# eriq-augustine/KB2E

Hardware: AMD Instinct MI355X
Metric: training triples/sec (1/2/4/8 MI355X) + FB15k Hits@10(Filter) (higher is better)
Workload: dtype f64

## Files before the change

kb2e_amd/csrc/engine.hip:

```cpp
#include <hip/hip_runtime.h>
#include <hip/hip_ext.h>
#include <hipcub/hipcub.hpp>

#include <algorithm>
#include <cmath>
#include <cstdio>
#include <cstring>
#include <map>
#include <memory>
#include <stdexcept>
#include <string>
#include <vector>

#include "../../include/kb2e_engine.h"
#include "glibc_rand.hpp"
#include "hip_util.hpp"
#include "eval.hpp"
#include "predict.hpp"
#include "classify.hpp"
#include "host_data.hpp"
#include "kernels_common.hpp"
#include "kernels_index.hpp"
#include "kernels_transe.hpp"
#include "kernels_transe_long.hpp"
// ... 1606 lines not shown
            for (int g = 0; g < 2; ++g) {
                fprintf(stderr, "fold_prof %d", g);
                for (int k = 0; k < 16; ++k) fprintf(stderr, " %llu", fp[g][k]);
                fprintf(stderr, "\n");
            }
            std::memset(fp, 0, sizeof(fp));
            HIPCHK(hipMemcpyToSymbol(HIP_SYMBOL(g_fold_prof), fp, sizeof(fp)));
            HIPCHK(hipMemcpyFromSymbol(fp[0], HIP_SYMBOL(g_long_prof), sizeof(fp[0])));
            fprintf(stderr, "long_prof");
            for (int k = 0; k < 16; ++k) fprintf(stderr, " %llu", fp[0][k]);
            fprintf(stderr, "\n");
            HIPCHK(hipMemcpyToSymbol(HIP_SYMBOL(g_long_prof), fp[1], sizeof(fp[1])));
        }
#endif
        if (getenv("KB2E_RPAR_STATS")) {
            unsigned long long st[16];
            HIPCHK(hipMemcpyFromSymbol(st, HIP_SYMBOL(g_rpar_rounds), sizeof(st)));
            cons_wave_take_stats(st);
            fprintf(stderr, "rpar_rounds rounds of row blocks %llu, tiles with violators %llu, most rounds of a block %llu\n",
                    st[0], st[1], st[2]);
            fprintf(stderr, "rpar_cons cycles: setup %llu, P0+rounds %llu, records %llu, longest block %llu, blocks %llu\n",
                    st[3], st[4], st[5], st[6], st[7]);
            if (c->rpar_cons_seq || c->rpar_cons_wide) {
                unsigned long long q[64];
                cons_seq_take_stats(q);
                fprintf(stderr, "rpar_cons chunk kernel: relations %llu, chunks %llu (most in a relation %llu), "
                        "violators %llu, rounds %llu (most %llu), cycles mean %.0f max %llu\n", q[0], q[1], q[6], q[2],
                        q[3], q[7], q[0] ? (double)q[4] / (double)q[0] : 0.0, q[5]);
                if (c->rpar_cons_wide && cons_chainw_pipelined(c->n))
                    fprintf(stderr, "rpar_cons pipelined wide chain phases (walker: prologue+K0, window list, walk, "
                            "B1 wait, row stores+fold, B2 wait, drain, window flags, tail, write-back+records, -; helper: "
                            "debt+fold+B2, X tile, B1 wait; walker: row+V, sums+rounds+g, later rows):");
                else if (c->rpar_cons_wide)
                    fprintf(stderr, "rpar_cons wide chain phases (prologue, window list, rows+barrier, P+Gram+B1, "
                            "K0, V+sums, B(1), rounds+g, B(2), later pairs, B(3), records+W update, chunk barrier, "
                            "window flags, tail, write-back):");
                else
                    fprintf(stderr, "rpar_cons chunk phases (prologue, chunk start, walk end + publish, B1 wait, "
                            "pick + row to LDS, helper B1 wait, after B1, V, sums, rounds + g, g store, later rows; helper wave 1: debt, tiles, "
                            "helper_sync wait, rows + corrections):");
                for (int k = 8; k < 24; ++k) fprintf(stderr, " %llu", q[k]);
                fprintf(stderr, "; hot relations (%llu, %llu chunks, %llu violators):", q[41], q[40], q[42]);
                for (int k = 24; k < 40; ++k) fprintf(stderr, " %llu", q[k]);
                if (c->rpar_cons_seq) {
                    fprintf(stderr, "; tail (last debt + barrier, slices to LDS + barrier, records, W write-back):");
                    for (int k = 44; k < 48; ++k) fprintf(stderr, " %llu", q[k]);
                    fprintf(stderr, "; hot tail:");
                    for (int k = 48; k < 52; ++k) fprintf(stderr, " %llu", q[k]);
                    fprintf(stderr, "; hot cycles %llu", q[43]);
                }
                fprintf(stderr, "\n");
            }
            if (c->rpar_cons_wave)
                fprintf(stderr, "rpar_cons wave kernel: longest setup %llu, P0+rounds %llu, records %llu, a wave's "
                        "rounds %llu; MFMA rounds before the VALU tail %llu, blocks entering it %llu\n",
                        st[8], st[9], st[10], st[11], st[12], st[13]);
            else
                fprintf(stderr, "rpar_rounds wave 0: loads+mfma issue %llu, barriers %llu, update part %llu, lockstep "
                        "rounds %llu, tail %llu, G+ballot %llu\n", st[8], st[9], st[10], st[11], st[12], st[13]);
            std::memset(st, 0, sizeof(st));
            HIPCHK(hipMemcpyToSymbol(HIP_SYMBOL(g_rpar_rounds), st, sizeof(st)));
        }
        if (loss) *loss = c->acc_loss;
        if (active) *active = c->acc_active;
        c->acc_loss = 0;
        c->acc_active = 0;
        return KB2E_OK;
    });
}

kb2e_status kb2e_train_epoch(kb2e_ctx* c, double* loss, int64_t* active) {
    return guarded(c, [&] {
// ... 288 lines not shown
```

kb2e_amd/csrc/engine_transr_parallel.inc:

```
namespace {

constexpr int32_t kRParLongMin = 128;

template <typename T, bool P, bool G>
const void* tile_fn(int nb) {
    switch (nb) {
        case 1: return (const void*)transr_tile_mfma_kernel<T, P, G, 1>;
        case 2: return (const void*)transr_tile_mfma_kernel<T, P, G, 2>;
        case 3: return (const void*)transr_tile_mfma_kernel<T, P, G, 3>;
        case 4: return (const void*)transr_tile_mfma_kernel<T, P, G, 4>;
        case 5: return (const void*)transr_tile_mfma_kernel<T, P, G, 5>;
        case 6: return (const void*)transr_tile_mfma_kernel<T, P, G, 6>;
        case 7: return (const void*)transr_tile_mfma_kernel<T, P, G, 7>;
        case 8: return (const void*)transr_tile_mfma_kernel<T, P, G, 8>;
    }
    throw std::runtime_error("TransR tile kernel: n > 128");
}

template <typename T>
const void* cons_tile_fn(int nb) {
    switch (nb) {
        case 1: return (const void*)transr_cons_tile_kernel<T, 1>;
        case 2: return (const void*)transr_cons_tile_kernel<T, 2>;
        case 3: return (const void*)transr_cons_tile_kernel<T, 3>;
// ... 269 lines not shown
        d.ne = c->cfg.num_entities;
        d.B = (int32_t)c->B;
        d.kl = c->kl;
        d.si = c->si_[set].as<int32_t>();
        d.sj = c->sj_[set].as<int32_t>();
        d.side = c->side_[set].as<uint8_t>();
        d.heads = c->heads.as<int32_t>();
        d.tails = c->tails.as<int32_t>();
        d.batch_t0 = c->rpar_batch_t0.as<int32_t>();
        d.td_r = c->rpar_td_r.as<int32_t>();
        d.td_cnt = c->rpar_td_cnt.as<int32_t>();
        d.td_kk = c->rpar_td_kk.as<int32_t>();
        d.td_ent = c->rpar_td_ent.as<int32_t>();
        rtile_desc_kernel<<<2048, 256, 0, st>>>(d);
        HIPCHK(hipGetLastError());
    }
}

DevBuf& buf_set(int set, DevBuf& s0, DevBuf& s1) { return set ? s1 : s0; }

bool sub_overlap_on() {
    const char* e = getenv("KB2E_SUB_OVERLAP");
    return !(e && e[0] == '0');
}

template <typename T>
void fill_rpar(kb2e_ctx* c, int64_t b, int j, int set, RParArgs& a, RParBufs<T>& bf) {
    const int64_t ib = b * c->sub + j;
    const int64_t first = b * c->B + (int64_t)j * c->Bs;
    const int64_t cnt = std::min<int64_t>(c->Bs, c->B - (int64_t)j * c->Bs);
    a = RParArgs{};
    a.heads = c->heads.as<int32_t>();
    a.tails = c->tails.as<int32_t>();
    a.rels = c->rels.as<int32_t>();
    a.si = c->si() + first;
    a.sj = c->sj() + first;
    a.side = c->side() + first;
    a.B = (int32_t)cnt;
    a.n = c->n;
    a.ld = c->ld;
    a.ne = c->cfg.num_entities;
    a.nr = c->cfg.num_relations;
    a.St = c->rpar_St;
    a.tgroup = c->rpar_tgroup;
    a.batch = (int32_t)ib;
    a.lr = c->cfg.learning_rate;
// ... 26 lines not shown
    bf.W = c->w.as<T>();
    bf.x = buf_set(set, c->xreal, c->sb_x).as<T>();
    bf.d = buf_set(set, c->aux, c->sb_d).as<T>();
    bf.y = buf_set(set, c->rpar_y, c->sb_y).as<T>();
    bf.wpart = buf_set(set, c->rpar_wpart, c->sb_wpart).as<T>();
    bf.rpart = buf_set(set, c->rpar_rpart, c->sb_rpart).as<T>();
    bf.pair = c->rpar_pair.as<T>();
    bf.relpair = c->rpar_relpair.as<T>();
    bf.relpair_stamp = c->rpar_relpair_stamp.as<uint32_t>();
    bf.err = c->dataflow_err.as<uint32_t>() + 1;
    if (c->rpar_mfma) {
        bf.pflag = buf_set(set, c->rpar_pflag, c->sb_pflag).as<uint8_t>();
        bf.cons_tile = buf_set(set, c->rpar_cons_tile, c->sb_cons_tile).as<int32_t>();
        bf.cons_ppt = c->rpar_cons_wave ? kConsPpt : 1;
        bf.cpairs = buf_set(set, c->rpar_cpairs, c->sb_cpairs).as<int32_t>();
        bf.vio = buf_set(set, c->rpar_vio, c->sb_vio).as<int32_t>();
        bf.cnrows = buf_set(set, c->rpar_cnrows, c->sb_cnrows).as<int32_t>();
        bf.stats = getenv("KB2E_RPAR_STATS") != nullptr;
        bf.last_renorm = c->rpar_cons_seq ? 1 : 0;
        if (const char* dbg = getenv("KB2E_CONS_DBG")) bf.dbg = atoi(dbg);
        if (const char* cl = getenv("KB2E_RPAR_CHAIN_LIST")) bf.chain_list = std::max(64, atoi(cl));
        if (const char* ct = getenv("KB2E_RPAR_CHAIN_TILES")) bf.chain_tiles = std::max(1, atoi(ct));
        if (const char* rc = getenv("KB2E_RPAR_REC_CAP")) bf.rec_cap = std::max(4, atoi(rc));
    }
    if (c->rpar_cons_wide || c->rpar_cons_gen || c->rpar_widep) {
        bf.pflag = buf_set(set, c->rpar_pflag, c->sb_pflag).as<uint8_t>();
        if (const char* dbg = getenv("KB2E_CONS_DBG")) bf.dbg = atoi(dbg);
        bf.stats = getenv("KB2E_RPAR_STATS") != nullptr;
        bf.last_renorm = 1;
    }
}

template <typename T>
void transr_phase_b(kb2e_ctx* c, RParArgs a, RParBufs<T> bf);

template <typename T>
void run_subbatch_transr_parallel(kb2e_ctx* c, int64_t b, int j) {
    const bool ov = c->sub > 1 && sub_overlap_on();
    const bool side = ov && j > 0;
    const int set = ov ? (j & 1) : 0;
    hipStream_t sa = side ? c->suba_stream : c->stream;
    RParArgs a;
    RParBufs<T> bf;
    fill_rpar<T>(c, b, j, set, a, bf);
    {
        unsigned long long* t0 = c->rpar_ptab.as<unsigned long long>();
// ... 225 lines not shown
```

kb2e_amd/csrc/kernels_transr_parallel.hpp:

```cpp
#pragma once

#include <type_traits>

#include "kernels_common.hpp"

namespace kb2e {

struct RTile {
    int32_t seg, q;
};

struct RParArgs {
    const int32_t* heads;
    const int32_t* tails;
    const int32_t* rels;
    const int32_t* si;
    const int32_t* sj;
    const uint8_t* side;
    int32_t B, n, ld, ne, nr, St;
    int32_t batch;
    int32_t tgroup;
    double lr, margin;
    int32_t compat, l1;
    const uint64_t* keys;
// ... 121 lines not shown
    T* ent;
    T* rel;
    T* W;
    T* x;
    T* d;
    T* y;
    T* wpart;
    T* rpart;
    T* pair;
    T* relpair;
    uint32_t* relpair_stamp;
    uint32_t stamp;
    uint8_t* pflag;
    int32_t* cons_tile;
    int32_t cons_ppt;
    int32_t* cpairs;
    int32_t* cnrows;
    int32_t stats;
    int32_t last_renorm;
    int32_t dbg;
    int32_t chain_list;
    int32_t chain_tiles;
    int32_t rec_cap;
    int32_t* vio;
    uint32_t* err;
};

__host__ __device__ constexpr int rm_up16_host_dev(int v) { return (v + 15) & ~15; }
constexpr int kCPairs = 64;

struct RParMerge {
    int32_t sub;
    int32_t Bs;
    int32_t Blast;
    int32_t tcap;
    int32_t nch;
    int32_t brel_cap;
};

template <typename P>
__host__ __device__ __forceinline__ void rpar_advance(P*& p, int64_t k) {
    if (p) p += k;
}

template <typename T>
__host__ __device__ __forceinline__ void rpar_sub_view(RParArgs& a, RParBufs<T>& bf, const RParMerge& m, int j) {
    const int64_t s0 = (int64_t)j * m.Bs, t0 = (int64_t)j * m.tcap;
    a.B = j == m.sub - 1 ? m.Blast : m.Bs;
    a.batch += j;
// ... 1030 lines not shown
```

kb2e_amd/csrc/kernels_transr_pipe.hpp:

```cpp
#pragma once

#include "kernels_transr_cons.hpp"
#include "kernels_transr_seq.hpp"

namespace kb2e {

constexpr int kPipeList = 1536;

template <typename T>
__host__ __device__ constexpr size_t pipe_lds(int n) {
    return sizeof(T) * ((size_t)rm_np(n) * rm_ld(n) + 5 * (size_t)kChainRows * rm_ld(n) +
                        3 * (size_t)kChainRows * (kChainRows + 1) + 4 * kChainRows + 4 * (size_t)rm_np(n)) +
           sizeof(int) * (size_t)(2 * kPipeList + kSeqMaxTiles + 1 + 8 + 2 * kChainRows);
}

constexpr int kRecGroup = 32;
constexpr int kRecReads = 8;

template <typename T, int NP, int L, int STAGE>
__device__ __forceinline__ void pipe_records(const RParArgs& a, const RParBufs<T>& bf, int r, const int32_t* vio,
                                             int nvt, const T* Wc, T* stage, int* slots, const int* slist,
                                             int nslist) {
    typedef T T2 __attribute__((ext_vector_type(2)));
    constexpr int NW = kChainThreads / kWave;
    constexpr int CAPW = STAGE / (NW * NP);
    static_assert(CAPW >= 1 && NW * CAPW <= kPipeList, "the record slots borrow a window list");
    static_assert(NP % 4 == 0 && (L * sizeof(T)) % 16 == 0 && (NP * sizeof(T)) % 16 == 0, "16-byte LDS reads");
    const int n = a.n, ld = a.ld, w = threadIdx.x >> 6, l = lane_id();
    const int nmine = nvt > w ? (nvt - w + NW - 1) / NW : 0;
    if (nmine == 0) return;
    const int capw = bf.rec_cap >= NW && bf.rec_cap < NW * CAPW ? bf.rec_cap / NW : CAPW;
    T* gs = stage + w * (CAPW * NP);
    int* sl = slots + w * CAPW;
    auto row_of = [&](int s) { return s >= 0 ? bf.pair + (int64_t)s * ld : bf.relpair + (int64_t)r * ld; };
    T wr[NP];
    {
        const T2* w2 = (const T2*)(Wc + (l < NP ? l : 0) * L);
#pragma unroll
        for (int q = 0; q < NP / 2; ++q) {
            const T2 x = w2[q];
            wr[2 * q] = x.x;
            wr[2 * q + 1] = x.y;
        }
    }
    for (int m0 = 0; m0 < nmine; m0 += capw) {
        const int cnt = nmine - m0 < capw ? nmine - m0 : capw;
        for (int i = l; i < cnt; i += kWave) {
            const int k = w + NW * (m0 + i);
            sl[i] = k < nslist ? slist[k] : vio[k];
        }
        wave_lds_sync();
        for (int i0 = 0; i0 < cnt; i0 += kRecGroup) {
            const int iu = i0 + (l & (kRecGroup - 1));
            const int sv = sl[iu < cnt ? iu : cnt - 1];
            T g[kRecGroup];
#pragma unroll
            for (int u = 0; u < kRecGroup; ++u) g[u] = row_of(__builtin_amdgcn_readlane(sv, u))[l < n ? l : 0];
            if (l < NP) {
#pragma unroll
                for (int u = 0; u < kRecGroup; ++u)
                    gs[(i0 + u < cnt ? i0 + u : cnt - 1) * NP + l] = l < n ? g[u] : T(0);
            }
        }
        wave_lds_sync();
        constexpr int NG = (NP / 2 + kRecReads - 1) / kRecReads, LA = NG >= 2 ? 2 : 1;
        T2 gr[NP / 2];
        auto g_load = [&](int i, int gq) {
            const T2* g2 = (const T2*)(gs + i * NP);
#pragma unroll
            for (int q = gq * kRecReads; q < (gq + 1) * kRecReads && q < NP / 2; ++q) gr[q] = g2[q];
        };
#pragma unroll
        for (int gq = 0; gq < LA; ++gq) g_load(0, gq);
        for (int i = 0; i < cnt; ++i) {
            T* row = row_of(sl[i]);
            const int inext = i + 1 < cnt ? i + 1 : i;
            T acc[4] = {T(0), T(0), T(0), T(0)};
            __builtin_amdgcn_sched_barrier(0);
#pragma unroll
            for (int gq = 0; gq < NG; ++gq) {
#pragma unroll
                for (int q = gq * kRecReads; q < (gq + 1) * kRecReads && q < NP / 2; ++q) {
                    acc[(2 * q) & 3] = fma(wr[2 * q], gr[q].x, acc[(2 * q) & 3]);
                    acc[(2 * q + 1) & 3] = fma(wr[2 * q + 1], gr[q].y, acc[(2 * q + 1) & 3]);
                }
                __builtin_amdgcn_sched_barrier(0);
                if (gq + LA < NG) g_load(i, gq + LA);
                else g_load(inext, gq + LA - NG);
                __builtin_amdgcn_sched_barrier(0);
            }
            T da = (acc[0] + acc[1]) + (acc[2] + acc[3]);
            asm volatile("" : "+v"(da));
            if (l < n) row[l] = -(T)a.lr * da;
        }
        wave_lds_sync();
    }
}

template <typename T, int KS, bool STATS>
__global__ __launch_bounds__(kChainThreads) void transr_cons_pipe_kernel(RParArgs a, RParBufs<T> bf) {
    using M = Mfma16<T>;
    static_assert(sizeof(T) == 8, "the D-row / k-step identity below is the FP64 fragment layout");
    constexpr int NB = (4 * KS + 15) / 16;
    constexpr int NP = 16 * NB, L = NP + 2, R = kChainRows, LG = R + 1;
    constexpr int NH = 2 * KS;
    constexpr int NSW = (NB + 2) / 3;
    static_assert(2 * R * L >= NP * L, "the K0 image borrows the two P buffers");
    static_assert(NSW * KS <= 4 * KS, "the helpers' slices share the walk's K0 registers");
    const int t0 = a.batch_t0[a.batch], t1 = a.batch_t0[a.batch + 1];
    int g0, r;
    if (!chain_first_tile(a, t0, t1, g0, r)) return;
    const int n = a.n, ld = a.ld;
    const int w = threadIdx.x >> 6, l = lane_id(), kq = l >> 4, l16 = l & 15;
    const bool mine = w < NB;
    const int col = 16 * w + l16;
    const int hw = w - 1;
    const T lr = (T)a.lr;
    extern __shared__ __attribute__((aligned(16))) char smem[];
    T* Wc = (T*)smem;
    T* Abuf = Wc + NP * L;
    T* Pbuf = Abuf + 3 * R * L;
    T* Gbuf = Pbuf + 2 * R * L;
    T* Cx = Gbuf + 2 * R * LG;
    int* slist = (int*)Cx;
    constexpr int kSlist = 2 * R * LG;
    T* qpart = Cx + R * LG;
    T* rp = qpart + 4 * R;
    int* pe = (int*)(rp + 4 * NP);
    int* ps = pe + kPipeList;
    int* pre = ps + kPipeList;
    int* misc = pre + kSeqMaxTiles + 1;
    int* vlist = misc + 8;
    const long long ck0 = STATS ? clock64() : 0;
    int n_chunks = 0;
    unsigned long long n_vio = 0, n_rounds = 0, max_m = 0;
    __shared__ unsigned long long ph[STATS ? 20 : 1];
    if (STATS && threadIdx.x < 20) ph[threadIdx.x] = 0;
    long long tq = ck0;
    auto tick = [&](int k) {
        if constexpr (STATS) {
            if (threadIdx.x == ((k >= 12 && k < 16) || k == 5 ? 64u : 0u)) {
                const long long t = clock64();
                ph[k] += (unsigned long long)(t - tq);
                tq = t;
            }
        }
    };

    for (int idx = threadIdx.x; idx < NP * NP; idx += kChainThreads) {
        const int j = idx / NP, i = idx % NP;
        Wc[j * L + i] = (j < n && i < n) ? bf.W[((int64_t)r * n + j) * ld + i] : T(0);
    }
    if (w == 0) {
        int run = 0;
        for (int m0 = 0;; m0 += kWave) {
            const int g = g0 + m0 + l;
            const uint64_t b = __ballot(t0 + g < t1 && a.td_r[t0 + g] == r);
            const int k = b == ~0ull ? kWave : __builtin_ctzll(~b);
            run += k;
            if (k < kWave) break;
        }
        const int c0 = bf.cnrows[g0] & 127;
        const int rel = c0 > 0 && bf.cpairs[(int64_t)g0 * 2 * kCPairs + kCPairs + c0 - 1] == -2;
        int kl = -1, gt = -1;
        for (int g = g0 + run - 1; g >= g0 && kl < 0; --g) {
            const int cs = a.td_cnt[t0 + g] & 255;
            const int kk = l < cs ? a.td_kk[(t0 + g) * 8 + l] : -1;
            const uint64_t b = __ballot(kk >= 0 && a.act[kk]);
            if (b) {
                kl = __shfl(kk, 63 - __builtin_clzll(b));
// ... 44 lines not shown
            for (int i = 0; i < 4 * KS; ++i) reg[i] = T(0);
#pragma unroll
            for (int si = 0; si < NSW; ++si) {
                const int cb = hw + 3 * si;
                if (cb < NB) {
#pragma unroll
                    for (int s = 0; s < KS; ++s) reg[si * KS + s] = Wc[(4 * s + kq) * L + cb * 16 + l16];
                }
            }
        }
        if (threadIdx.x == 0) {
            misc[5] = 0;
            misc[6] = -1;
            misc[7] = -1;
        }
        __syncthreads();
    }
    bool changed = false;
    int32_t* const vio = bf.vio + (int64_t)g0 * kCPairs;
    int nvt = 0;
    int pend_nv = 0, pend_par = 0, pend_pc = 0, pend_ka = 0;
    tick(0);

    auto gram_tile = [&](const T* Ar, const T* Bm, int rt, int cb, T* out, int ldo) {
        typename M::acc_t acc = {T(0), T(0), T(0), T(0)};
        T av[KS], bv[KS];
#pragma unroll
        for (int s = 0; s < KS; ++s) {
            av[s] = Ar[(rt * 16 + l16) * L + 4 * s + kq];
            bv[s] = Bm[(cb * 16 + l16) * L + 4 * s + kq];
        }
#pragma unroll
        for (int s = 0; s < KS; ++s) acc = M::mma(av[s], bv[s], acc);
#pragma unroll
        for (int q = 0; q < 4; ++q) out[(rt * 16 + kq + 4 * q) * ldo + cb * 16 + l16] = acc[q];
    };
    auto proj_tile = [&](const T* Ar, int rt, int si, T* out) {
        const int cb = hw + 3 * si;
        typename M::acc_t acc = {T(0), T(0), T(0), T(0)};
        T av[KS];
#pragma unroll
        for (int s = 0; s < KS; ++s) av[s] = Ar[(rt * 16 + l16) * L + 4 * s + kq];
#pragma unroll
        for (int s = 0; s < KS; ++s) acc = M::mma(av[s], reg[si * KS + s], acc);
#pragma unroll
        for (int q = 0; q < 4; ++q) out[(rt * 16 + kq + 4 * q) * L + cb * 16 + l16] = acc[q];
    };
    constexpr int kHT = kChainThreads - kWave;
    constexpr int kRowsPer = (R * NP + kHT - 1) / kHT;
    static_assert(kRowsPer <= 32, "rows_ok bits");
    const int ht = (int)threadIdx.x - kWave;
    T rows[kRowsPer];
    uint32_t rows_ok = 0;
    auto load_rows = [&](int b, int e) {
        if (w == 0) return;
        int ent[kRowsPer];
#pragma unroll
        for (int q = 0; q < kRowsPer; ++q) {
            const int f = b + (ht + q * kHT) / NP;
            ent[q] = pe[f < kPipeList ? f : kPipeList - 1];
        }
        rows_ok = 0;
#pragma unroll
        for (int q = 0; q < kRowsPer; ++q) {
            const int idx = ht + q * kHT;
// ... 6 lines not shown
    auto store_rows = [&](int slot) {
        if (w == 0) return;
#pragma unroll
        for (int q = 0; q < kRowsPer; ++q) {
            const int idx = ht + q * kHT;
            if (idx < R * NP) Abuf[slot * R * L + (idx / NP) * L + idx % NP] = ((rows_ok >> q) & 1) ? rows[q] : T(0);
        }
    };
    int hsync_target = 0;
    auto helper_sync = [&]() {
        hsync_target += kChainThreads / kWave - 1;
        if (l == 0 && !((bf.dbg & 32) && hw == 0))
            __hip_atomic_fetch_add(&misc[5], 1, __ATOMIC_RELEASE, __HIP_MEMORY_SCOPE_WORKGROUP);
        for (uint32_t sp = 0;
             __hip_atomic_load(&misc[5], __ATOMIC_ACQUIRE, __HIP_MEMORY_SCOPE_WORKGROUP) < hsync_target; ++sp) {
            if (sp > (1u << 22)) {
                if (l == 0) __hip_atomic_store(bf.err, 1u, __ATOMIC_RELAXED, __HIP_MEMORY_SCOPE_AGENT);
                break;
            }
            __builtin_amdgcn_s_sleep(1);
        }
    };
    auto chunk_outputs = [&](T* Pn, int cn, const T* Pc, const T* An, const T* Ac, const int* vl, int ck, int base,
                             int cc, int vpar) {
        constexpr int NE = NP / 16, NPS = (R + 11) / 12;
        const int rs = ht >> 4, cb = (ht & 15) * NE;
        T x[NPS][NE];
#pragma unroll
        for (int p = 0; p < NPS; ++p) {
            const int j = rs + 12 * p;
#pragma unroll
            for (int u = 0; u < NE; ++u) x[p][u] = j < cn ? Pn[j * L + cb + u] : T(0);
        }
        int used = 0;
        for (uint32_t sp = 0;; ++sp) {
            const bool done = __hip_atomic_load(&misc[6], __ATOMIC_ACQUIRE, __HIP_MEMORY_SCOPE_WORKGROUP) == ck;
            const int pw = __hip_atomic_load(&misc[7], __ATOMIC_ACQUIRE, __HIP_MEMORY_SCOPE_WORKGROUP);
            const int avail = (pw >> 6) == ck ? (pw & 63) : 0;
            for (; used < avail; ++used) {
                const int v = vl[used];
                const int slv = ps[base + v];
                T gv[NE], av[NE], d[NPS];
#pragma unroll
                for (int u = 0; u < NE; ++u) {
                    gv[u] = Pc[v * L + cb + u];
                    av[u] = Ac[v * L + cb + u];
                }
                if (cn > 0) {
#pragma unroll
                    for (int p = 0; p < NPS; ++p) {
                        const int j = rs + 12 * p;
                        d[p] = T(0);
#pragma unroll
                        for (int u = 0; u < NE; ++u) d[p] = fma(j < R ? An[j * L + cb + u] : T(0), av[u], d[p]);
                    }
                    row16_sums<T, NPS>(d);
#pragma unroll
                    for (int p = 0; p < NPS; ++p) {
                        const int j = rs + 12 * p;
                        if (j < cn) {
                            const T gl = -lr * d[p];
#pragma unroll
                            for (int u = 0; u < NE; ++u) x[p][u] = fma(gl, gv[u], x[p][u]);
                        }
                    }
                }
                if (rs == 0) {
                    T* dst = slv >= 0 ? bf.pair + (int64_t)slv * ld : bf.relpair + (int64_t)r * ld;
#pragma unroll
                    for (int u = 0; u < NE; ++u)
                        if (cb + u < n) dst[cb + u] = gv[u];
                    if (ht == 0) {
                        vio[nvt + used] = slv;
                        if (nvt + used < kSlist) slist[nvt + used] = slv;
                    }
                }
            }
            if (done) {
                if (ht < cc) {
                    const int sl = ps[base + ht];
                    const bool vio_l = ((uint32_t)misc[1 + 2 * vpar] >> ht) & 1;
                    if (sl >= 0) bf.pflag[sl] = vio_l ? 1 : 0;
                    else if (vio_l) bf.relpair_stamp[r] = bf.stamp;
                }
                break;
            }
            if (sp > (1u << 22)) {
                if (l == 0) __hip_atomic_store(bf.err, 1u, __ATOMIC_RELAXED, __HIP_MEMORY_SCOPE_AGENT);
                break;
            }
            __builtin_amdgcn_s_sleep(1);
        }
        if (cn == 0) return;
        T sq[NPS];
#pragma unroll
        for (int p = 0; p < NPS; ++p) {
            const int j = rs + 12 * p;
            sq[p] = T(0);
            if (j < cn) {
#pragma unroll
                for (int u = 0; u < NE; ++u) {
                    if (used) Pn[j * L + cb + u] = x[p][u];
                    sq[p] = fma(x[p][u], x[p][u], sq[p]);
                }
            }
        }
        row16_sums<T, NPS>(sq);
        if ((ht & 15) == 0) {
#pragma unroll
            for (int p = 0; p < NPS; ++p) {
                const int j = rs + 12 * p;
                if (j < R) {
                    qpart[j] = j < cn ? sq[p] : T(0);
                    for (int v = 1; v < NB; ++v) qpart[v * R + j] = T(0);
                }
            }
        }
    };
    auto correct_q = [&](T* Pn, int cn, int nv, const T* Pc, const int* vl) {
        constexpr int NE = NP / 8;
        const int j = threadIdx.x >> 3, cb = (threadIdx.x & 7) * NE;
        T sq = T(0);
        if (j < cn) {
            T x[NE];
#pragma unroll
            for (int u = 0; u < NE; ++u) x[u] = Pn[j * L + cb + u];
            for (int k = 0; k < nv; ++k) {
                const int v = vl[k];
                const T gl = -lr * Cx[j * LG + v];
#pragma unroll
                for (int u = 0; u < NE; ++u) x[u] = fma(gl, Pc[v * L + cb + u], x[u]);
            }
#pragma unroll
            for (int u = 0; u < NE; ++u) {
                if (nv) Pn[j * L + cb + u] = x[u];
                sq = fma(x[u], x[u], sq);
            }
        }
        sq += dpp_mov<0xB1>(sq);
        sq += dpp_mov<0x4E>(sq);
// ... 1 lines not shown
        if ((threadIdx.x & 7) == 0) {
            qpart[j] = j < cn ? sq : T(0);
            for (int v = 1; v < NB; ++v) qpart[v * R + j] = T(0);
        }
    };
    auto apply_pending = [&]() {
        if (w == 0 || pend_nv == 0) return;
        const T* Pp = Pbuf + pend_pc * R * L;
        const T* Ap = Abuf + pend_ka * R * L;
        const int* vl = vlist + pend_par * R;
        const int vmine = l < pend_nv ? vl[l] : 0;
        T an[KS], gn[NSW];
        auto ldv = [&](int k) {
            const int v = __builtin_amdgcn_readlane(vmine, k);
#pragma unroll
            for (int s = 0; s < KS; ++s) an[s] = Ap[v * L + 4 * s + kq];
#pragma unroll
            for (int si = 0; si < NSW; ++si) {
                const int cb = hw + 3 * si;
                gn[si] = cb < NB ? -lr * Pp[v * L + cb * 16 + l16] : T(0);
            }
        };
        const int nvu = (bf.dbg & 16) ? 0 : pend_nv;
        if (nvu > 0) ldv(0);
        for (int k = 0; k < nvu; ++k) {
            T ac[KS], gc[NSW];
#pragma unroll
            for (int s = 0; s < KS; ++s) ac[s] = an[s];
#pragma unroll
            for (int si = 0; si < NSW; ++si) gc[si] = gn[si];
            if (k + 1 < nvu) ldv(k + 1);
#pragma unroll
            for (int si = 0; si < NSW; ++si)
                if (hw + 3 * si < NB) {
#pragma unroll
                    for (int s = 0; s < KS; ++s) reg[si * KS + s] = fma(ac[s], gc[si], reg[si * KS + s]);
                }
        }
    };
    auto renorm = [&] {
        if (w > 0) {
#pragma unroll
            for (int si = 0; si < NSW; ++si) {
                const int cb = hw + 3 * si;
#pragma unroll
                for (int s = 0; s < KS; ++s) {
// ... 5 lines not shown
        }
        __syncthreads();
        if (w > 0) {
#pragma unroll
            for (int si = 0; si < NSW; ++si) {
                if (hw + 3 * si >= NB) continue;
#pragma unroll
                for (int s = 0; s < KS; ++s) {
                    const int jr = 4 * s + kq;
                    T ss = rp[jr];
                    for (int v = 1; v < NB; ++v) ss += rp[v * NP + jr];
                    if (jr < n) reg[si * KS + s] = reg[si * KS + s] / sqrt(ss);
                }
            }
        }
        __syncthreads();
    };
    auto fresh = [&](const T* A, int cc, T* P, T* G) {
        const int nrt = cc > 16 ? 2 : 1;
        if (w > 0) {
#pragma unroll
            for (int si = 0; si < NSW; ++si)
                if (hw + 3 * si < NB)
                    for (int rt = 0; rt < nrt; ++rt) proj_tile(A, rt, si, P);
        } else {
            for (int gi = 0; gi < (nrt == 2 ? 3 : 1); ++gi) gram_tile(A, A, gi == 0 ? 0 : 1, gi == 2 ? 1 : 0, G, LG);
        }
        __syncthreads();
        correct_q(P, cc, 0, nullptr, vlist);
        __syncthreads();
    };

    const int tile_cap = bf.chain_tiles >= 1 && bf.chain_tiles < kSeqMaxTiles ? bf.chain_tiles : kSeqMaxTiles;
    const int list_cap = bf.chain_list >= 64 && bf.chain_list < kPipeList ? bf.chain_list : kPipeList;
    int pc = 0;
    int par = 0;
    for (int gw = g0; gw < g0 + run || gw == g0;) {
        if (w == 0) {
            const int nt = g0 + run - gw < tile_cap ? g0 + run - gw : tile_cap;
            int carry = 0, fit = 0;
            for (int m0 = 0; m0 < nt; m0 += kWave) {
                const int g = m0 + l;
                int c = g < nt ? (bf.cnrows[gw + g] & 127) : 0;
                if (gw + g == g0 && has_rel) c -= 1;
                int x = c;
#pragma unroll
                for (int s = 1; s < kWave; s <<= 1) {
                    const int y = __shfl_up(x, s);
                    if (l >= s) x += y;
// ... 26 lines not shown
                e = cp[f - pre[lo]];
                sl = cp[kCPairs + f - pre[lo]];
            }
            pe[f] = e;
            ps[f] = sl;
        }
        auto chunk_end = [&](int b) {
            return b < tail_start ? (b + R < tail_start ? b + R : tail_start) : npairs;
        };
        __syncthreads();
        if (npairs > 0) {
            const int e0 = chunk_end(0);
            const int e1 = e0 < npairs ? chunk_end(e0) : e0;
            load_rows(0, e0);
            store_rows(0);
            load_rows(e0, e1);
            store_rows(1);
            load_rows(e1, e1 < npairs ? chunk_end(e1) : e1);
            if (tail_start == 0 && changed) renorm();
            __syncthreads();
            pc = 0;
            fresh(Abuf, e0, Pbuf, Gbuf);
        }
        int ka = 0;
        for (int base = 0; base < npairs;) {
            const int nbase = chunk_end(base);
            const int cc = nbase - base;
            const int nb2 = nbase < npairs ? chunk_end(nbase) : nbase;
            const int cn = nb2 - nbase;
            const T* A = Abuf + ka * R * L;
            const T* An = Abuf + (ka == 2 ? 0 : ka + 1) * R * L;
            T* P = Pbuf + pc * R * L;
            T* Pn = Pbuf + (pc ^ 1) * R * L;
            T* Gm = Gbuf + pc * R * LG;
            T* Gn = Gbuf + (pc ^ 1) * R * LG;
            int* vl = vlist + par * R;
            const int ck = n_chunks;
            ++n_chunks;
            tick(1);
            if (w == 0) {
                const int j = l & (R - 1);
                T q = T(0);
                if (j < cc) {
                    q = qpart[j];
                    for (int v = 1; v < NB; ++v) q += qpart[v * R + j];
                }
// ... 97 lines not shown
                                               __HIP_MEMORY_SCOPE_WORKGROUP);
                        }
                        ++npub;
                        vmask |= 1u << v;
                        cursor = v + 1;
                        if constexpr (STATS) ++n_vio;
                        tick(11);
                    }
                }
                if (l == 0) {
                    misc[1 + 2 * par] = (int)vmask;
                    misc[2 + 2 * par] = npub;
                    __hip_atomic_store(&misc[6], ck, __ATOMIC_RELEASE, __HIP_MEMORY_SCOPE_WORKGROUP);
                }
                tick(2);
            } else {
                apply_pending();
                tick(12);
                if (cn > 0) {
                    const int nrt = cn > 16 ? 2 : 1, crt = cc > 16 ? 2 : 1;
#pragma unroll
                    for (int si = 0; si < NSW; ++si)
                        if (hw + 3 * si < NB)
                            for (int rt = 0; rt < nrt; ++rt) proj_tile(An, rt, si, Pn);
                    const int ng = nrt == 2 ? 3 : 1;
                    int load[3];
#pragma unroll
                    for (int h = 0; h < 3; ++h) load[h] = nrt * ((NB - h + 2) / 3);
                    for (int tl = 0; tl < ng; ++tl) {
                        int best = 0;
#pragma unroll
                        for (int h = 1; h < 3; ++h) best = load[h] < load[best] ? h : best;
                        ++load[best];
                        if (best == hw) gram_tile(An, An, tl == 0 ? 0 : 1, tl == 2 ? 1 : 0, Gn, LG);
                    }
                    (void)crt;
                }
                tick(13);
                helper_sync();
                tick(14);
                if (nb2 < npairs || cn > 0) {
                    store_rows(ka == 0 ? 2 : ka - 1);
                    const int n3 = nb2 < npairs ? chunk_end(nb2) : nb2;
                    load_rows(n3, n3 < npairs ? chunk_end(n3) : n3);
                }
                chunk_outputs(Pn, cn, P, An, A, vl, ck, base, cc, par);
                tick(15);
            }
            __syncthreads();
            tick(w == 0 ? 3 : 5);
            const uint32_t vmask = (uint32_t)misc[1 + 2 * par];
            const int nv = misc[2 + 2 * par];
            pend_nv = nv;
            pend_par = par;
            pend_pc = pc;
            pend_ka = ka;
            nvt += nv;
            if (vmask) changed = true;
            const bool restart = nbase == tail_start && changed && cn > 0;
            tick(6);
            if (restart) {
                apply_pending();
                pend_nv = 0;
                __syncthreads();
                renorm();
                fresh(An, cn, Pn, Gn);
            }
            pc ^= 1;
            par ^= 1;
            ka = ka == 2 ? 0 : ka + 1;
            base = nbase;
        }
        apply_pending();
        pend_nv = 0;
        __syncthreads();
        tick(16);
        gw += ntile;
        if (last || gw >= g0 + run) break;
    }
    if (w > 0) {
#pragma unroll
        for (int si = 0; si < NSW; ++si) {
            const int cb = hw + 3 * si;
            if (cb < NB) {
#pragma unroll
                for (int s = 0; s < KS; ++s) Wc[(4 * s + kq) * L + cb * 16 + l16] = reg[si * KS + s];
            }
        }
    }
    __syncthreads();
    tick(17);
    pipe_records<T, NP, L, 5 * R * L>(a, bf, r, vio, nvt, Wc, Abuf, pe, slist, kSlist);
    if constexpr (STATS) {
        __syncthreads();
        tick(18);
    }
    {
        constexpr int NWB = NP * NP / kChainThreads;
        static_assert(NWB * kChainThreads == NP * NP, "whole rounds of the write-back");
        T wv[NWB];
#pragma unroll
        for (int q = 0; q < NWB; ++q) {
            const int idx = threadIdx.x + q * kChainThreads;
            wv[q] = Wc[(idx / NP) * L + idx % NP];
        }
#pragma unroll
        for (int q = 0; q < NWB; ++q) {
            const int idx = threadIdx.x + q * kChainThreads;
            const int jj = idx / NP, i = idx % NP;
            if (jj < n && i < n) bf.W[((int64_t)r * n + jj) * ld + i] = wv[q];
        }
    }
    if constexpr (STATS) {
        tick(19);
        if (threadIdx.x == 0) {
            const unsigned long long cyc = (unsigned long long)(clock64() - ck0);
            atomicAdd(&g_seq_stats[0], 1ull);
            atomicAdd(&g_seq_stats[1], (unsigned long long)n_chunks);
            atomicAdd(&g_seq_stats[2], n_vio);
            atomicAdd(&g_seq_stats[3], n_rounds);
            atomicAdd(&g_seq_stats[4], cyc);
            atomicMax(&g_seq_stats[5], cyc);
            atomicMax(&g_seq_stats[6], (unsigned long long)n_chunks);
            atomicMax(&g_seq_stats[7], max_m);
            for (int k = 0; k < 16; ++k) atomicAdd(&g_seq_stats[8 + k], ph[k]);
            for (int k = 0; k < 4; ++k) atomicAdd(&g_seq_stats[44 + k], ph[16 + k]);
            if (n_chunks >= 12) {
                for (int k = 0; k < 16; ++k) atomicAdd(&g_seq_stats[24 + k], ph[k]);
                atomicAdd(&g_seq_stats[40], (unsigned long long)n_chunks);
                atomicAdd(&g_seq_stats[41], 1ull);
                atomicAdd(&g_seq_stats[42], n_vio);
                atomicAdd(&g_seq_stats[43], cyc);
                for (int k = 0; k < 4; ++k) atomicAdd(&g_seq_stats[48 + k], ph[16 + k]);
            }
        }
    }
}

}
```

kb2e_amd/csrc/kernels_transr_seq.hpp:

```cpp
#pragma once

#include "kernels_transr_mfma.hpp"

namespace kb2e {

constexpr int kChainRows = 32;
constexpr int kChainThreads = 256;
constexpr int kSeqMaxTiles = 256;

static __device__ unsigned long long g_seq_stats[64];

template <typename T, int K>
__device__ __forceinline__ void row16_sums(T (&v)[K]) {
#pragma unroll
    for (int k = 0; k < K; ++k) v[k] += dpp_ror<8>(v[k]);
#pragma unroll
    for (int k = 0; k < K; ++k) v[k] += dpp_ror<4>(v[k]);
#pragma unroll
    for (int k = 0; k < K; ++k) v[k] += dpp_ror<2>(v[k]);
#pragma unroll
    for (int k = 0; k < K; ++k) v[k] += dpp_ror<1>(v[k]);
}

template <typename T, int K>
__device__ __forceinline__ void wave_sums(T (&v)[K]) {
    row16_sums<T, K>(v);
#pragma unroll
    for (int k = 0; k < K; ++k) v[k] += dpp_mov<kDppBcast15>(v[k]);
#pragma unroll
    for (int k = 0; k < K; ++k) v[k] += dpp_mov<kDppBcast31>(v[k]);
#pragma unroll
    for (int k = 0; k < K; ++k) v[k] = readlane_f(v[k], 63);
}
// ... 82 lines not shown
```

kb2e_amd/csrc/transr_cons.hip:

```cpp
#include "transr_cons.hpp"

#include <algorithm>
#include <cstring>
#include <stdexcept>
#include <string>
#include <utility>

#include "hip_util.hpp"
#include "kernels_transr_cons.hpp"
#include "kernels_transr_seq.hpp"
#include "kernels_transr_chainw.hpp"
#include "kernels_transr_chainwp.hpp"
#include "kernels_transr_chaing.hpp"
#include "kernels_transr_pipe.hpp"
#include "kernels_transr_wave.hpp"

namespace kb2e {

namespace {

enum Kind { kCons, kGrad, kProj, kGradMerged, kProjMerged };

int chain_grid(const RParArgs& a) { return a.nrel > 0 ? a.nrel : 1; }

// ... 178 lines not shown
    RParArgs aa = a;
    RParBufs<T> bb = bf;
    void* args[] = {&aa, &bb};
    HIPCHK(hipLaunchKernel((const void*)transr_cons_chain_gen_kernel<T>, dim3(chain_grid(a)), dim3(kGenThreads), args,
                           lds, stream));
}
template void cons_chaing_launch<double>(const RParArgs&, const RParBufs<double>&, size_t, hipStream_t);
template void cons_chaing_launch<float>(const RParArgs&, const RParBufs<float>&, size_t, hipStream_t);

template void proj_wave_launch<double>(const RParArgs&, const RParBufs<double>&, int, hipStream_t);
template void proj_wave_launch<float>(const RParArgs&, const RParBufs<float>&, int, hipStream_t);

template void grad_wave_launch<double>(const RParArgs&, const RParBufs<double>&, int, hipStream_t);
template void grad_wave_launch<float>(const RParArgs&, const RParBufs<float>&, int, hipStream_t);

template void proj_wave_merged_launch<double>(const RParArgs&, const RParBufs<double>&, const RParMerge&, hipStream_t);
template void proj_wave_merged_launch<float>(const RParArgs&, const RParBufs<float>&, const RParMerge&, hipStream_t);
template void grad_wave_merged_launch<double>(const RParArgs&, const RParBufs<double>&, const RParMerge&, hipStream_t);
template void grad_wave_merged_launch<float>(const RParArgs&, const RParBufs<float>&, const RParMerge&, hipStream_t);

template void cons_wave_launch<double>(const RParArgs&, const RParBufs<double>&, int, size_t, hipStream_t);
template void cons_wave_launch<float>(const RParArgs&, const RParBufs<float>&, int, size_t, hipStream_t);

void cons_seq_take_stats(unsigned long long (&st)[64]) {
    HIPCHK(hipMemcpyFromSymbol(st, HIP_SYMBOL(g_seq_stats), sizeof(st)));
    unsigned long long z[64] = {};
    HIPCHK(hipMemcpyToSymbol(HIP_SYMBOL(g_seq_stats), z, sizeof(z)));
}

void cons_wave_take_stats(unsigned long long (&st)[16]) {
    unsigned long long mine[16];
    HIPCHK(hipMemcpyFromSymbol(mine, HIP_SYMBOL(g_cons_stats), sizeof(mine)));
    for (int k = 0; k < 16; ++k) st[k] = (k == 2 || k == 6) ? std::max(st[k], mine[k]) : st[k] + mine[k];
    std::memset(mine, 0, sizeof(mine));
    HIPCHK(hipMemcpyToSymbol(HIP_SYMBOL(g_cons_stats), mine, sizeof(mine)));
}

}
```

kb2e_amd/csrc/transr_cons.hpp:

```cpp
#pragma once

#include <hip/hip_runtime.h>

#include "kernels_transr_parallel.hpp"

namespace kb2e {

constexpr int kWideMaxN = 112;
constexpr int kConsPpt = 1;

bool cons_wave_supported(int n);
size_t cons_wave_setup(int n, int St, int esize);
template <typename T>
void cons_wave_launch(const RParArgs& a, const RParBufs<T>& bf, int grid, size_t lds, hipStream_t stream);
template <typename T>
void proj_wave_launch(const RParArgs& a, const RParBufs<T>& bf, int grid, hipStream_t stream);
template <typename T>
void grad_wave_launch(const RParArgs& a, const RParBufs<T>& bf, int grid, hipStream_t stream);
template <typename T>
void proj_wave_merged_launch(const RParArgs& a, const RParBufs<T>& bf, const RParMerge& m, hipStream_t stream);
template <typename T>
void grad_wave_merged_launch(const RParArgs& a, const RParBufs<T>& bf, const RParMerge& m, hipStream_t stream);
size_t cons_seq_setup(int n);
void cons_seq_launch(const RParArgs& a, const RParBufs<double>& bf, size_t lds, hipStream_t stream);
bool cons_chainw_supported(int n);
size_t cons_chainw_setup(int n);
void cons_chainw_launch(const RParArgs& a, const RParBufs<double>& bf, size_t lds, hipStream_t stream);
bool cons_chaing_supported(int n);
size_t cons_chaing_setup(int n, int esize);
template <typename T>
void cons_chaing_launch(const RParArgs& a, const RParBufs<T>& bf, size_t lds, hipStream_t stream);
bool cons_chainw_pipelined(int n);
void cons_seq_take_stats(unsigned long long (&st)[64]);
void cons_wave_take_stats(unsigned long long (&st)[16]);

constexpr int kWideParMaxN = 512;
struct WideGeom {
    int St = 1;
    int chunk = 2;
    size_t tile_lds = 0, scan_lds = 0, chain_lds = 0;
};
bool wide_par_supported(int n);
WideGeom wide_setup(int n, int ld, int esize);
template <typename T>
void wide_phase_a(const RParArgs& a, const RParBufs<T>& bf, const WideGeom& g, int tgrid, double* scan,
                  double* scan_pre, const double* work_in, double* work_out, hipStream_t st);
template <typename T>
void wide_phase_b(const RParArgs& a, const RParBufs<T>& bf, const WideGeom& g, double* wsc, bool constraint,
                  int rel_segs_max, hipStream_t st);

}
```

Before: 9.449 million.

## Streamline pipelined chain handover: preload An rows, defer flags, double-buffer corrections

Adds an on-by-default pipe_opt handover mode to the pipelined TransR constraint chain kernel. The helper wave preloads its An slices into registers before polling, instead of re-reading LDS for every violator. It also stops zeroing extra qpart slots and moves the pflag/stamp writes out of the polling loop into a post-barrier step. The pending-violator correction loop is double-buffered so loads overlap FMAs, and sched barriers are placed in the MFMA tiles. Extra stats phases are added for profiling, at the cost of more register pressure and a changed write ordering for the flags.

```diff
diff --git a/kb2e_amd/csrc/engine.hip b/kb2e_amd/csrc/engine.hip
--- a/kb2e_amd/csrc/engine.hip
+++ b/kb2e_amd/csrc/engine.hip
@@ -1652,7 +1652,7 @@
             fprintf(stderr, "rpar_cons cycles: setup %llu, P0+rounds %llu, records %llu, longest block %llu, blocks %llu\n",
                     st[3], st[4], st[5], st[6], st[7]);
             if (c->rpar_cons_seq || c->rpar_cons_wide) {
-                unsigned long long q[64];
+                unsigned long long q[96];
                 cons_seq_take_stats(q);
                 fprintf(stderr, "rpar_cons chunk kernel: relations %llu, chunks %llu (most in a relation %llu), "
                         "violators %llu, rounds %llu (most %llu), cycles mean %.0f max %llu\n", q[0], q[1], q[6], q[2],
@@ -1678,6 +1678,11 @@
                     fprintf(stderr, "; hot tail:");
                     for (int k = 48; k < 52; ++k) fprintf(stderr, " %llu", q[k]);
                     fprintf(stderr, "; hot cycles %llu", q[43]);
+                    fprintf(stderr, "; hot outside the violator loop (window set-up; B1 wait at 0, 1-2, 3-5, 6+ "
+                            "violators, chunks of each; helper wave 1 after helper_sync without polling: after the walk's "
+                            "end, row staging + P_n loads, corrections + outputs; records on wave 0: W row, slot lists, "
+                            "G loads issue, arrival + staging, record loops):");
+                    for (int k = 52; k < 69; ++k) fprintf(stderr, " %llu", q[k]);
                 }
                 fprintf(stderr, "\n");
             }
diff --git a/kb2e_amd/csrc/engine_transr_parallel.inc b/kb2e_amd/csrc/engine_transr_parallel.inc
--- a/kb2e_amd/csrc/engine_transr_parallel.inc
+++ b/kb2e_amd/csrc/engine_transr_parallel.inc
@@ -315,6 +315,11 @@
 bool sub_overlap_on() {
     const char* e = getenv("KB2E_SUB_OVERLAP");
     return !(e && e[0] == '0');
+}
+
+int32_t pipe_opt_bits() {
+    const char* e = getenv("KB2E_RPAR_PIPE_OPT");
+    return e && e[0] ? (int32_t)(atoi(e) & kPipeOptAll) : kPipeOptAll;
 }
 
 template <typename T>
@@ -387,6 +392,7 @@
         if (const char* cl = getenv("KB2E_RPAR_CHAIN_LIST")) bf.chain_list = std::max(64, atoi(cl));
         if (const char* ct = getenv("KB2E_RPAR_CHAIN_TILES")) bf.chain_tiles = std::max(1, atoi(ct));
         if (const char* rc = getenv("KB2E_RPAR_REC_CAP")) bf.rec_cap = std::max(4, atoi(rc));
+        bf.pipe_opt = pipe_opt_bits();
     }
     if (c->rpar_cons_wide || c->rpar_cons_gen || c->rpar_widep) {
         bf.pflag = buf_set(set, c->rpar_pflag, c->sb_pflag).as<uint8_t>();
diff --git a/kb2e_amd/csrc/kernels_transr_parallel.hpp b/kb2e_amd/csrc/kernels_transr_parallel.hpp
--- a/kb2e_amd/csrc/kernels_transr_parallel.hpp
+++ b/kb2e_amd/csrc/kernels_transr_parallel.hpp
@@ -167,9 +167,12 @@
     int32_t chain_list;
     int32_t chain_tiles;
     int32_t rec_cap;
+    int32_t pipe_opt;
     int32_t* vio;
     uint32_t* err;
 };
+
+constexpr int32_t kPipeOptHandover = 2, kPipeOptAll = kPipeOptHandover;
 
 __host__ __device__ constexpr int rm_up16_host_dev(int v) { return (v + 15) & ~15; }
 constexpr int kCPairs = 64;
diff --git a/kb2e_amd/csrc/kernels_transr_pipe.hpp b/kb2e_amd/csrc/kernels_transr_pipe.hpp
--- a/kb2e_amd/csrc/kernels_transr_pipe.hpp
+++ b/kb2e_amd/csrc/kernels_transr_pipe.hpp
@@ -1,4 +1,6 @@
 #pragma once
+
+#include <type_traits>
 
 #include "kernels_transr_cons.hpp"
 #include "kernels_transr_seq.hpp"
@@ -17,10 +19,10 @@
 constexpr int kRecGroup = 32;
 constexpr int kRecReads = 8;
 
-template <typename T, int NP, int L, int STAGE>
+template <typename T, int NP, int L, int STAGE, bool STATS>
 __device__ __forceinline__ void pipe_records(const RParArgs& a, const RParBufs<T>& bf, int r, const int32_t* vio,
                                              int nvt, const T* Wc, T* stage, int* slots, const int* slist,
-                                             int nslist) {
+                                             int nslist, unsigned long long* ph) {
     typedef T T2 __attribute__((ext_vector_type(2)));
     constexpr int NW = kChainThreads / kWave;
     constexpr int CAPW = STAGE / (NW * NP);
@@ -29,6 +31,16 @@
     const int n = a.n, ld = a.ld, w = threadIdx.x >> 6, l = lane_id();
     const int nmine = nvt > w ? (nvt - w + NW - 1) / NW : 0;
     if (nmine == 0) return;
+    long long tq = STATS ? clock64() : 0;
+    auto tick = [&](int k) {
+        if constexpr (STATS) {
+            if (threadIdx.x == 0) {
+                const long long t = clock64();
+                ph[k] += (unsigned long long)(t - tq);
+                tq = t;
+            }
+        }
+    };
     const int capw = bf.rec_cap >= NW && bf.rec_cap < NW * CAPW ? bf.rec_cap / NW : CAPW;
     T* gs = stage + w * (CAPW * NP);
     int* sl = slots + w * CAPW;
@@ -43,6 +55,13 @@
             wr[2 * q + 1] = x.y;
         }
     }
+    if constexpr (STATS) {
+        T sink = T(0);
+#pragma unroll
+        for (int q = 0; q < NP; ++q) sink += wr[q];
+        asm volatile("" ::"v"(sink));
+    }
+    tick(0);
     for (int m0 = 0; m0 < nmine; m0 += capw) {
         const int cnt = nmine - m0 < capw ? nmine - m0 : capw;
         for (int i = l; i < cnt; i += kWave) {
@@ -50,17 +69,24 @@
             sl[i] = k < nslist ? slist[k] : vio[k];
         }
         wave_lds_sync();
+        tick(1);
         for (int i0 = 0; i0 < cnt; i0 += kRecGroup) {
             const int iu = i0 + (l & (kRecGroup - 1));
             const int sv = sl[iu < cnt ? iu : cnt - 1];
             T g[kRecGroup];
 #pragma unroll
             for (int u = 0; u < kRecGroup; ++u) g[u] = row_of(__builtin_amdgcn_readlane(sv, u))[l < n ? l : 0];
+            if constexpr (STATS) {
+                __builtin_amdgcn_sched_barrier(0);
+                tick(2);
+                __builtin_amdgcn_sched_barrier(0);
+            }
             if (l < NP) {
 #pragma unroll
                 for (int u = 0; u < kRecGroup; ++u)
                     gs[(i0 + u < cnt ? i0 + u : cnt - 1) * NP + l] = l < n ? g[u] : T(0);
             }
+            tick(3);
         }
         wave_lds_sync();
         constexpr int NG = (NP / 2 + kRecReads - 1) / kRecReads, LA = NG >= 2 ? 2 : 1;
@@ -94,6 +120,7 @@
             if (l < n) row[l] = -(T)a.lr * da;
         }
         wave_lds_sync();
+        tick(4);
     }
 }
 
@@ -134,18 +161,21 @@
     const long long ck0 = STATS ? clock64() : 0;
     int n_chunks = 0;
     unsigned long long n_vio = 0, n_rounds = 0, max_m = 0;
-    __shared__ unsigned long long ph[STATS ? 20 : 1];
-    if (STATS && threadIdx.x < 20) ph[threadIdx.x] = 0;
-    long long tq = ck0;
+    constexpr int kPh = 40;
+    __shared__ unsigned long long ph[STATS ? kPh : 1];
+    if (STATS && threadIdx.x < kPh) ph[threadIdx.x] = 0;
+    long long tq = ck0, dtq = 0;
     auto tick = [&](int k) {
         if constexpr (STATS) {
             if (threadIdx.x == ((k >= 12 && k < 16) || k == 5 ? 64u : 0u)) {
                 const long long t = clock64();
-                ph[k] += (unsigned long long)(t - tq);
+                dtq = t - tq;
+                ph[k] += (unsigned long long)dtq;
                 tq = t;
             }
         }
     };
+    const bool o_hand = (bf.pipe_opt & kPipeOptHandover) != 0;
 
     for (int idx = threadIdx.x; idx < NP * NP; idx += kChainThreads) {
         const int j = idx / NP, i = idx % NP;
@@ -236,7 +266,7 @@
     int pend_nv = 0, pend_par = 0, pend_pc = 0, pend_ka = 0;
     tick(0);
 
-    auto gram_tile = [&](const T* Ar, const T* Bm, int rt, int cb, T* out, int ldo) {
+    auto gram_tile = [&](const T* Ar, const T* Bm, int rt, int cb, T* out, int ldo, auto ahead) {
         typename M::acc_t acc = {T(0), T(0), T(0), T(0)};
         T av[KS], bv[KS];
 #pragma unroll
@@ -244,17 +274,19 @@
             av[s] = Ar[(rt * 16 + l16) * L + 4 * s + kq];
             bv[s] = Bm[(cb * 16 + l16) * L + 4 * s + kq];
         }
+        if constexpr (decltype(ahead)::value) __builtin_amdgcn_sched_barrier(0);
 #pragma unroll
         for (int s = 0; s < KS; ++s) acc = M::mma(av[s], bv[s], acc);
 #pragma unroll
         for (int q = 0; q < 4; ++q) out[(rt * 16 + kq + 4 * q) * ldo + cb * 16 + l16] = acc[q];
     };
-    auto proj_tile = [&](const T* Ar, int rt, int si, T* out) {
+    auto proj_tile = [&](const T* Ar, int rt, int si, T* out, auto ahead) {
         const int cb = hw + 3 * si;
         typename M::acc_t acc = {T(0), T(0), T(0), T(0)};
         T av[KS];
 #pragma unroll
         for (int s = 0; s < KS; ++s) av[s] = Ar[(rt * 16 + l16) * L + 4 * s + kq];
+        if constexpr (decltype(ahead)::value) __builtin_amdgcn_sched_barrier(0);
 #pragma unroll
         for (int s = 0; s < KS; ++s) acc = M::mma(av[s], reg[si * KS + s], acc);
 #pragma unroll
@@ -307,7 +339,7 @@
         }
     };
     auto chunk_outputs = [&](T* Pn, int cn, const T* Pc, const T* An, const T* Ac, const int* vl, int ck, int base,
-                             int cc, int vpar) {
+                             int cc, int vpar, long long t_sync) {
         constexpr int NE = NP / 16, NPS = (R + 11) / 12;
         const int rs = ht >> 4, cb = (ht & 15) * NE;
         T x[NPS][NE];
@@ -317,11 +349,31 @@
 #pragma unroll
             for (int u = 0; u < NE; ++u) x[p][u] = j < cn ? Pn[j * L + cb + u] : T(0);
         }
+        T anr[NPS][NE];
+#pragma unroll
+        for (int p = 0; p < NPS; ++p) {
+            const int j = rs + 12 * p;
+#pragma unroll
+            for (int u = 0; u < NE; ++u) anr[p][u] = o_hand && cn > 0 && j < R ? An[j * L + cb + u] : T(0);
+        }
         int used = 0;
+        long long tw = 0;
+        if constexpr (STATS) {
+            if (threadIdx.x == 64u) {
+                T sink = T(0);
+#pragma unroll
+                for (int p = 0; p < NPS; ++p)
+#pragma unroll
+                    for (int u = 0; u < NE; ++u) sink += x[p][u];
+                asm volatile("" ::"v"(sink));
+                ph[30] += (unsigned long long)(clock64() - t_sync);
+            }
+        }
         for (uint32_t sp = 0;; ++sp) {
             const bool done = __hip_atomic_load(&misc[6], __ATOMIC_ACQUIRE, __HIP_MEMORY_SCOPE_WORKGROUP) == ck;
             const int pw = __hip_atomic_load(&misc[7], __ATOMIC_ACQUIRE, __HIP_MEMORY_SCOPE_WORKGROUP);
             const int avail = (pw >> 6) == ck ? (pw & 63) : 0;
+            if constexpr (STATS) tw = clock64();
             for (; used < avail; ++used) {
                 const int v = vl[used];
                 const int slv = ps[base + v];
@@ -336,8 +388,13 @@
                     for (int p = 0; p < NPS; ++p) {
                         const int j = rs + 12 * p;
                         d[p] = T(0);
-#pragma unroll
-                        for (int u = 0; u < NE; ++u) d[p] = fma(j < R ? An[j * L + cb + u] : T(0), av[u], d[p]);
+                        if (o_hand) {
+#pragma unroll
+                            for (int u = 0; u < NE; ++u) d[p] = fma(anr[p][u], av[u], d[p]);
+                        } else {
+#pragma unroll
+                            for (int u = 0; u < NE; ++u) d[p] = fma(j < R ? An[j * L + cb + u] : T(0), av[u], d[p]);
+                        }
                     }
                     row16_sums<T, NPS>(d);
 #pragma unroll
@@ -361,8 +418,13 @@
                     }
                 }
             }
+            if constexpr (STATS) {
+                const long long t = clock64();
+                if (threadIdx.x == 64u) ph[31] += (unsigned long long)(t - tw);
+                tw = t;
+            }
             if (done) {
-                if (ht < cc) {
+                if (!o_hand && ht < cc) {
                     const int sl = ps[base + ht];
                     const bool vio_l = ((uint32_t)misc[1 + 2 * vpar] >> ht) & 1;
                     if (sl >= 0) bf.pflag[sl] = vio_l ? 1 : 0;
@@ -376,7 +438,12 @@
             }
             __builtin_amdgcn_s_sleep(1);
         }
-        if (cn == 0) return;
+        auto post = [&] {
+            if constexpr (STATS) {
+                if (threadIdx.x == 64u) ph[29] += (unsigned long long)(clock64() - tw);
+            }
+        };
+        if (cn == 0) return post();
         T sq[NPS];
 #pragma unroll
         for (int p = 0; p < NPS; ++p) {
@@ -397,10 +464,19 @@
                 const int j = rs + 12 * p;
                 if (j < R) {
                     qpart[j] = j < cn ? sq[p] : T(0);
-                    for (int v = 1; v < NB; ++v) qpart[v * R + j] = T(0);
-                }
-            }
-        }
+                    if (!o_hand)
+                        for (int v = 1; v < NB; ++v) qpart[v * R + j] = T(0);
+                }
+            }
+        }
+        post();
+    };
+    auto chunk_flags = [&](int base, int cc, uint32_t vmask) {
+        if (w == 0 || ht >= cc) return;
+        const int sl = ps[base + ht];
+        const bool vio_l = (vmask >> ht) & 1;
+        if (sl >= 0) bf.pflag[sl] = vio_l ? 1 : 0;
+        else if (vio_l) bf.relpair_stamp[r] = bf.stamp;
     };
     auto correct_q = [&](T* Pn, int cn, int nv, const T* Pc, const int* vl) {
         constexpr int NE = NP / 8;
@@ -448,6 +524,39 @@
             }
         };
         const int nvu = (bf.dbg & 16) ? 0 : pend_nv;
+        if (o_hand) {
+            T a0[KS], a1[KS], ga[NSW], gb[NSW];
+            auto ld2 = [&](int k, T(&av)[KS], T(&gv)[NSW]) {
+                const int v = __builtin_amdgcn_readlane(vmine, k);
+#pragma unroll
+                for (int s = 0; s < KS; ++s) av[s] = Ap[v * L + 4 * s + kq];
+#pragma unroll
+                for (int si = 0; si < NSW; ++si) {
+                    const int cb = hw + 3 * si;
+                    gv[si] = Pp[v * L + (cb < NB ? cb : 0) * 16 + l16];
+                }
+            };
+            auto fm2 = [&](const T(&av)[KS], const T(&gv)[NSW]) {
+#pragma unroll
+                for (int si = 0; si < NSW; ++si)
+                    if (hw + 3 * si < NB) {
+                        const T gc = -lr * gv[si];
+#pragma unroll
+                        for (int s = 0; s < KS; ++s) reg[si * KS + s] = fma(av[s], gc, reg[si * KS + s]);
+                    }
+            };
+            if (nvu > 0) ld2(0, a0, ga);
+            if (nvu > 1) ld2(1, a1, gb);
+            for (int k = 0; k < nvu; k += 2) {
+                fm2(a0, ga);
+                if (k + 2 < nvu) ld2(k + 2, a0, ga);
+                if (k + 1 < nvu) {
+                    fm2(a1, gb);
+                    if (k + 3 < nvu) ld2(k + 3, a1, gb);
+                }
+            }
+            return;
+        }
         if (nvu > 0) ldv(0);
         for (int k = 0; k < nvu; ++k) {
             T ac[KS], gc[NSW];
@@ -499,9 +608,10 @@
 #pragma unroll
             for (int si = 0; si < NSW; ++si)
                 if (hw + 3 * si < NB)
-                    for (int rt = 0; rt < nrt; ++rt) proj_tile(A, rt, si, P);
+                    for (int rt = 0; rt < nrt; ++rt) proj_tile(A, rt, si, P, std::false_type{});
         } else {
-            for (int gi = 0; gi < (nrt == 2 ? 3 : 1); ++gi) gram_tile(A, A, gi == 0 ? 0 : 1, gi == 2 ? 1 : 0, G, LG);
+            for (int gi = 0; gi < (nrt == 2 ? 3 : 1); ++gi)
+                gram_tile(A, A, gi == 0 ? 0 : 1, gi == 2 ? 1 : 0, G, LG, std::false_type{});
         }
         __syncthreads();
         correct_q(P, cc, 0, nullptr, vlist);
@@ -574,6 +684,7 @@
             pc = 0;
             fresh(Abuf, e0, Pbuf, Gbuf);
         }
+        tick(20);
         int ka = 0;
         for (int base = 0; base < npairs;) {
             const int nbase = chunk_end(base);
@@ -717,7 +828,10 @@
 #pragma unroll
                     for (int si = 0; si < NSW; ++si)
                         if (hw + 3 * si < NB)
-                            for (int rt = 0; rt < nrt; ++rt) proj_tile(An, rt, si, Pn);
+                            for (int rt = 0; rt < nrt; ++rt) {
+                                if (o_hand) proj_tile(An, rt, si, Pn, std::true_type{});
+                                else proj_tile(An, rt, si, Pn, std::false_type{});
+                            }
                     const int ng = nrt == 2 ? 3 : 1;
                     int load[3];
 #pragma unroll
@@ -727,25 +841,37 @@
 #pragma unroll
                         for (int h = 1; h < 3; ++h) best = load[h] < load[best] ? h : best;
                         ++load[best];
-                        if (best == hw) gram_tile(An, An, tl == 0 ? 0 : 1, tl == 2 ? 1 : 0, Gn, LG);
+                        if (best == hw) {
+                            if (o_hand) gram_tile(An, An, tl == 0 ? 0 : 1, tl == 2 ? 1 : 0, Gn, LG, std::true_type{});
+                            else gram_tile(An, An, tl == 0 ? 0 : 1, tl == 2 ? 1 : 0, Gn, LG, std::false_type{});
+                        }
                     }
                     (void)crt;
                 }
                 tick(13);
                 helper_sync();
                 tick(14);
+                const long long t_sync = STATS ? clock64() : 0;
                 if (nb2 < npairs || cn > 0) {
                     store_rows(ka == 0 ? 2 : ka - 1);
                     const int n3 = nb2 < npairs ? chunk_end(nb2) : nb2;
                     load_rows(n3, n3 < npairs ? chunk_end(n3) : n3);
                 }
-                chunk_outputs(Pn, cn, P, An, A, vl, ck, base, cc, par);
+                chunk_outputs(Pn, cn, P, An, A, vl, ck, base, cc, par, t_sync);
                 tick(15);
             }
             __syncthreads();
             tick(w == 0 ? 3 : 5);
             const uint32_t vmask = (uint32_t)misc[1 + 2 * par];
             const int nv = misc[2 + 2 * par];
+            if constexpr (STATS) {
+                if (threadIdx.x == 0) {
+                    const int bk = nv == 0 ? 0 : nv <= 2 ? 1 : nv <= 5 ? 2 : 3;
+                    ph[21 + bk] += (unsigned long long)dtq;
+                    ph[25 + bk] += 1;
+                }
+            }
+            if (o_hand) chunk_flags(base, cc, vmask);
             pend_nv = nv;
             pend_par = par;
             pend_pc = pc;
@@ -785,7 +911,7 @@
     }
     __syncthreads();
     tick(17);
-    pipe_records<T, NP, L, 5 * R * L>(a, bf, r, vio, nvt, Wc, Abuf, pe, slist, kSlist);
+    pipe_records<T, NP, L, 5 * R * L, STATS>(a, bf, r, vio, nvt, Wc, Abuf, pe, slist, kSlist, ph + (STATS ? 32 : 0));
     if constexpr (STATS) {
         __syncthreads();
         tick(18);
@@ -827,6 +953,7 @@
                 atomicAdd(&g_seq_stats[42], n_vio);
                 atomicAdd(&g_seq_stats[43], cyc);
                 for (int k = 0; k < 4; ++k) atomicAdd(&g_seq_stats[48 + k], ph[16 + k]);
+                for (int k = 20; k < 37; ++k) atomicAdd(&g_seq_stats[32 + k], ph[k]);
             }
         }
     }
diff --git a/kb2e_amd/csrc/kernels_transr_seq.hpp b/kb2e_amd/csrc/kernels_transr_seq.hpp
--- a/kb2e_amd/csrc/kernels_transr_seq.hpp
+++ b/kb2e_amd/csrc/kernels_transr_seq.hpp
@@ -8,7 +8,7 @@
 constexpr int kChainThreads = 256;
 constexpr int kSeqMaxTiles = 256;
 
-static __device__ unsigned long long g_seq_stats[64];
+static __device__ unsigned long long g_seq_stats[96];
 
 template <typename T, int K>
 __device__ __forceinline__ void row16_sums(T (&v)[K]) {
diff --git a/kb2e_amd/csrc/transr_cons.hip b/kb2e_amd/csrc/transr_cons.hip
--- a/kb2e_amd/csrc/transr_cons.hip
+++ b/kb2e_amd/csrc/transr_cons.hip
@@ -224,9 +224,9 @@
 template void cons_wave_launch<double>(const RParArgs&, const RParBufs<double>&, int, size_t, hipStream_t);
 template void cons_wave_launch<float>(const RParArgs&, const RParBufs<float>&, int, size_t, hipStream_t);
 
-void cons_seq_take_stats(unsigned long long (&st)[64]) {
+void cons_seq_take_stats(unsigned long long (&st)[96]) {
     HIPCHK(hipMemcpyFromSymbol(st, HIP_SYMBOL(g_seq_stats), sizeof(st)));
-    unsigned long long z[64] = {};
+    unsigned long long z[96] = {};
     HIPCHK(hipMemcpyToSymbol(HIP_SYMBOL(g_seq_stats), z, sizeof(z)));
 }
 
diff --git a/kb2e_amd/csrc/transr_cons.hpp b/kb2e_amd/csrc/transr_cons.hpp
--- a/kb2e_amd/csrc/transr_cons.hpp
+++ b/kb2e_amd/csrc/transr_cons.hpp
@@ -31,7 +31,7 @@
 template <typename T>
 void cons_chaing_launch(const RParArgs& a, const RParBufs<T>& bf, size_t lds, hipStream_t stream);
 bool cons_chainw_pipelined(int n);
-void cons_seq_take_stats(unsigned long long (&st)[64]);
+void cons_seq_take_stats(unsigned long long (&st)[96]);
 void cons_wave_take_stats(unsigned long long (&st)[16]);
 
 constexpr int kWideParMaxN = 512;
```

Result: faster. 9.725 million (median of 6 runs) (+2.9%).
